# yeyupiaoling/MASR

Hardware: AMD Instinct MI355X
Metric: audio-seconds/sec (RTF^-1), conformer_streaming_fbank b32x10s, PCM->fbank->encoder->ctc_greedy->text (higher is better)
Workload: dtype f32; 1 GPU; configs[1]: conformer.yml streaming fbank, batch=32 synthetic 16 kHz 10 s utterances per GPU, ctc_greedy, random-init weights V=4233; global_batch=32, parallelism=dp1, world_size_observed=1, backend=none

## Files before the change

### include/masr_hip.h

```cpp
#ifndef MASR_HIP_H
#define MASR_HIP_H
#include <stdint.h>
#ifdef __cplusplus
extern "C" {
#endif

typedef struct masr_engine masr_engine;

typedef struct masr_config {
    int32_t model_kind;
    int32_t d_model;
    int32_t heads;
    int32_t d_ff;
    int32_t num_blocks;
    int32_t cnn_kernel;
    int32_t n_mels;
    int32_t vocab_size;
    int32_t causal;
    int32_t max_pos;
    int32_t device_id;
    int32_t reserved[5];
} masr_config;

const char* masr_last_error(void);
// ... 132 lines not shown

int masr_resample_f32(const float* x, int64_t n_orig, double ratio, const double* win, const double* dwin, int64_t nwin,
                      int32_t num_table, float* y, int64_t n_out);
int masr_encode_chunk(masr_engine* e, const int32_t* stream_ids, int32_t n, const float* feats_dev, int32_t Tc,
                      float* probs_dev, int32_t* argmax_dev, float* maxprob_dev, void* stream);
int masr_stream_export_cache(masr_engine* e, int32_t stream_id, float* att_dev, float* cnn_dev, void* stream);

int masr_op_layernorm(masr_engine* e, const float* x_dev, const float* w_dev, const float* b_dev, float* y_dev,
                      int32_t M, float eps, void* stream);
int masr_op_gemm(masr_engine* e, const float* a_dev, const float* w_dev, const float* bias_dev, const float* res_dev,
                 float* c_dev, int32_t M, int32_t N, int32_t K, int32_t act, float alpha, void* stream);

#define MASR_SIDE_STREAMS 5
int masr_side_stream(masr_engine* e, int32_t kind, void** stream_out);

#define MASR_LANES 2
int masr_select_lane(masr_engine* e, int32_t lane);

int masr_debug_set(masr_engine* e, int32_t key, int32_t value);

int masr_profile_select(masr_engine* e, int32_t kind);
int masr_profile_read(masr_engine* e, double* total_ms, int64_t* launches, double* flops, int32_t reset);

#ifdef __cplusplus
}
#endif
#endif
```

### masr_amd/_lib.py

```python
import ctypes as C
import os

from .build import LIB_PATH

_lib = None


class MasrConfig(C.Structure):
    _fields_ = [('model_kind', C.c_int32), ('d_model', C.c_int32), ('heads', C.c_int32), ('d_ff', C.c_int32),
                ('num_blocks', C.c_int32), ('cnn_kernel', C.c_int32), ('n_mels', C.c_int32),
                ('vocab_size', C.c_int32), ('causal', C.c_int32), ('max_pos', C.c_int32), ('device_id', C.c_int32),
                ('reserved', C.c_int32 * 5)]


class MasrError(RuntimeError):
    pass


_P = C.c_void_p
_I = C.c_int32
_F = C.c_float

SIGNATURES = {
    'masr_last_error': [],
# ... 52 lines not shown
    'masr_pool_close': [_P, _I],
    'masr_pool_reset': [_P, _I],
    'masr_pool_step': [_P, _I, _P, _P, _P, _P, _P, _P, _P, C.POINTER(_I), C.POINTER(_P), C.POINTER(_P), C.POINTER(_P),
                       C.POINTER(_I), C.POINTER(_P), _P],
    'masr_pool_profile': [_P, C.POINTER(C.c_double), C.POINTER(C.c_int64), _I],
    'masr_encoder_frames': [_P, _I, C.POINTER(_I)],
    'masr_engine_info': [_P, C.POINTER(_I), C.POINTER(_I), C.POINTER(_I)],
    'masr_stream_open': [_P, _I, C.POINTER(_I)],
    'masr_stream_reset': [_P, _I],
    'masr_stream_close': [_P, _I],
    'masr_stream_offset': [_P, _I, C.POINTER(_I)],
    'masr_stream_cache_len': [_P, _I, C.POINTER(_I)],
    'masr_stream_room': [_P, _I, C.POINTER(_I)],
    'masr_resample_f32': [_P, C.c_int64, C.c_double, _P, _P, C.c_int64, _I, _P, C.c_int64],
    'masr_stream_set_history': [_P, _I, _I],
    'masr_encode_chunk': [_P, C.POINTER(_I), _I, _P, _I, _P, _P, _P, _P],
    'masr_stream_export_cache': [_P, _I, _P, _P, _P],
    'masr_op_layernorm': [_P, _P, _P, _P, _P, _I, _F, _P],
    'masr_op_gemm': [_P, _P, _P, _P, _P, _P, _I, _I, _I, _I, _F, _P],
    'masr_side_stream': [_P, _I, C.POINTER(_P)],
    'masr_select_lane': [_P, _I],
    'masr_stage_rows': [_P, C.c_int64, _P, _P, _I, _I, _I],
    'masr_debug_set': [_P, _I, _I],
    'masr_profile_select': [_P, _I],
    'masr_profile_read': [_P, C.POINTER(C.c_double), C.POINTER(C.c_int64), C.POINTER(C.c_double), _I],
}
_RESTYPE = {'masr_last_error': C.c_char_p, 'masr_destroy': None, 'masr_beam_destroy': None, 'masr_lm_destroy': None,
            'masr_lm_last_error': C.c_char_p, 'masr_vad_last_error': C.c_char_p, 'masr_vad_destroy': None, 'masr_pool_destroy': None}


GAIN_FN = C.CFUNCTYPE(C.c_int, C.POINTER(C.c_float), C.c_int32, C.c_float, C.POINTER(C.c_float), C.c_void_p)


def lib():
    global _lib
    if _lib is not None:
        return _lib
    import torch
    if not os.path.exists(LIB_PATH):
        raise MasrError(f'{LIB_PATH} not found: build it with `python -m masr_amd.build` '
                        f'(hipcc --offload-arch=gfx950). There is no CPU fallback.')
    h = C.CDLL(LIB_PATH)
    for name, args in SIGNATURES.items():
        fn = getattr(h, name)
        fn.argtypes = args
        fn.restype = _RESTYPE.get(name, C.c_int)
# ... 8 lines not shown
```

### masr_amd/csrc/common.h

```cpp
#pragma once
#include <hip/hip_runtime.h>
#include <stdint.h>

#include "lm_scorer.h"

#ifndef MASR_EXPERIMENTS
#define MASR_EXPERIMENTS 0
#endif

typedef float f32x4 __attribute__((ext_vector_type(4)));
typedef float f32x16 __attribute__((ext_vector_type(16)));

namespace masr {

struct LdsAttr {
    size_t granted[32] = {};
};
void ensure_dynamic_lds(const void* fn, size_t bytes, LdsAttr& st);
void note_launch_error(const char* what, hipError_t e);

#ifdef __HIPCC__
struct SeqRow {
    int b, t;
};
// ... 168 lines not shown
    const float* pre_lnb;
    long plane_stride;
    int seq_t, pad_t;
};
struct FfnHead {
    const float* glu;
    const float* dw_w;
    const float* dw_b;
    const float* lnw;
    const float* lnb;
    const float* gconst;
    const float* W;
    const float* bias;
    const int* lens;
    int seq_t, ktaps, mstride;
    float* xout;
};
int launch_ffn_fused(float* x, const float* lnw, const float* lnb, const float* w1, const float* b1, const float* w2,
                     const float* b2, int M, int dff, float eps, float scale, int affine_prologue, float* partial,
                     int nsplit, hipStream_t s, const FfnPostLn* post = nullptr, const FfnTail* tail = nullptr,
                     const FfnHead* head = nullptr, bool packed = false);
void launch_pack_ffn_pc(const float* w1, const float* w2, float* p1, float* p2, int dff, hipStream_t s);
void launch_pack_rows_pc(const float* w, float* p, int N, hipStream_t s, int n_src = -1);
struct SqzStageArgs {
    float* x;
    float* out;
    const float* att;
    const float* head_w;
    const float* head_b;
    const float *ln_a_w, *ln_a_b, *ln_b_w, *ln_b_b;
    const float *ffn_s, *ffn_b, *w1, *b1, *w2, *b2;
    const float *tail_w, *tail_b, *tail_s, *tail_sb;
    float* tail_out;
    float* glu_out;
    const float* glu;
    const float *dw_w, *dw_b, *bn_scale, *bn_shift, *gconst;
    const float* gpad;
    const int* lens;
    int M, dff, seq_t, mstride, ktaps, tail_n, glu_pad_l, glu_pad_tot;
    float eps;
    int skip_pad;
};
bool launch_sqz_stage(const SqzStageArgs& a, int stage, hipStream_t s);
#if MASR_EXPERIMENTS
int launch_ffn_dual(float* x, const float* lnw, const float* lnb, const float* p1, const float* b1, const float* p2,
                    const float* b2, int M, int dff, float eps, float scale, int affine_prologue, hipStream_t s,
// ... 134 lines not shown
```

### masr_amd/csrc/engine.hip

```cpp
#include <math.h>
#include <stdio.h>
#include <stdlib.h>
#include <string.h>

#include <map>
#include <mutex>
#include <string>
#include <vector>

#include "../../include/masr_hip.h"
#include "common.h"

using namespace masr;
namespace masr {
int lm_device_view(masr_lm* lm, LmView* out);
bool lm_word_based(const masr_lm* lm);
}
extern "C" const char* masr_lm_last_error(void);

static thread_local std::string g_err;
static int fail(const std::string& m) {
    g_err = m;
    return 1;
}
// ... 206 lines not shown
    int lane = 0;
    hipEvent_t pack_ev = nullptr;
    void* pack_stream = nullptr;
    bool pack_pending = false;
    bool finalized = false;
    std::map<std::string, HostTensor> host;
    std::vector<void*> owned;
    float *cmvn_mean = nullptr, *cmvn_istd = nullptr, *conv1_w = nullptr, *conv1_b = nullptr, *conv2_w = nullptr,
          *conv2_b = nullptr, *embed_w = nullptr, *embed_b = nullptr, *after_w = nullptr, *after_b = nullptr,
          *ctc_w = nullptr, *ctc_b = nullptr, *pe = nullptr;
    std::vector<LayerW> layers;
    std::vector<SqLayerW> sq_layers;
    std::vector<Ds2LayerW> ds2_layers;
    std::vector<GBeam> gbeams;
    DevBuf beam_pool, beam_state;
    std::map<void*, std::pair<DevBuf, DevBuf>> beam_ws;
    std::map<void*, DevBuf> ms_ws;
    int skip_padding = 7;
    void* beam_first_stream = nullptr;
    bool beam_first_set = false;
    std::map<const float*, std::pair<DevBuf, DevBuf>> ffn_packed;
    std::map<const float*, std::pair<DevBuf, DevBuf>> ffn_dual_packed;
    std::map<const float*, std::pair<DevBuf, DevBuf>> x3_packed;
    long long* beam_prof = nullptr;
    float *preln_w = nullptr, *preln_b = nullptr, *tr_dw_w = nullptr, *tr_dw_b = nullptr, *tr_pw_w = nullptr,
          *tr_pw_b = nullptr, *rec_w = nullptr, *rec_b = nullptr;
    int reduce_idx = -1, recover_idx = -1;
    int stride_idx = -1, n_group_layers = 0, group_size = 3;
    bool conv_bn = false;
    float *window = nullptr, *melwt = nullptr, *tw512 = nullptr, *twr4 = nullptr;
    FbankTables fbank_tables() const { return FbankTables{window, melwt, tw512, twr4, mel_lo}; }
    int* mel_lo = nullptr;
    float *dct = nullptr, *lifter = nullptr;
    int dct_ceps = 0;
    double *lin_win = nullptr, *lin_tw = nullptr;
    double lin_scale = 0.0;
    std::vector<Stream> streams;
    int prof_kind = 0;
    int prof_stride = 1, prof_seen = 0;
    std::vector<std::pair<hipEvent_t, hipEvent_t>> prof_events;
    size_t prof_used = 0;
    double prof_flops = 0.0;
};

namespace {

// ... 33 lines not shown
        on = e->prof_kind != 0 && (e->prof_kind == kind || (e->prof_kind == PROF_GEMM && (kind == PROF_FFN1 || kind == PROF_CONV2 || kind == PROF_FFN_TAIL || kind == PROF_FFN_HEAD)));
        if (on && e->prof_stride > 1) on = (e->prof_seen++ % e->prof_stride) == 0;
        if (!on) return;
        if (e->prof_used == e->prof_events.size()) {
            hipEvent_t a, b;
            hipEventCreate(&a);
            hipEventCreate(&b);
            e->prof_events.push_back({a, b});
        }
        hipEventRecord(e->prof_events[e->prof_used].first, s);
        e->prof_flops += flops;
    }
    ~ProfScope() {
        if (!on) return;
        hipEventRecord(e->prof_events[e->prof_used].second, s);
        e->prof_used++;
    }
};

struct CallGuard {
    masr_engine* e;
    hipStream_t s;
    size_t n0;
    static size_t packed_count(const masr_engine* e) { return e->ffn_packed.size() + e->ffn_dual_packed.size() + e->x3_packed.size(); }
    CallGuard(masr_engine* e_, hipStream_t s_) : e(e_), s(s_), n0(packed_count(e_)) {
        if (!e->pack_pending) return;
        if (hipEventQuery(e->pack_ev) == hipSuccess) {
            e->pack_pending = false;
        } else {
            (void)hipGetLastError();
            if ((void*)s != e->pack_stream) (void)hipStreamWaitEvent(s, e->pack_ev, 0);
        }
    }
    ~CallGuard() {
        if (packed_count(e) == n0) return;
        if (!e->pack_ev && hipEventCreateWithFlags(&e->pack_ev, hipEventDisableTiming) != hipSuccess) return;
        if (hipEventRecord(e->pack_ev, s) == hipSuccess) {
            e->pack_stream = (void*)s;
            e->pack_pending = true;
        }
    }
};

static int g_ffn_dual = 0;
static int g_ffn_packed = 2;
static int g_bf16x3 = 0;

void gemm(masr_engine* e, hipStream_t s, const float* A, int lda, const float* W, const float* bias, float* C, int ldc,
          int M, int N, int K, int act, float alpha, const float* R, int ldr, int kind = PROF_GEMM,
          const int* lens = nullptr, int mask_tp = 0) {
    GemmArgs a{};
    a.A = A; a.W = W; a.bias = bias; a.C = C; a.R = R; a.lens = lens;
    a.M = M; a.N = N; a.K = K; a.lda = lda; a.ldc = ldc; a.ldr = ldr;
    a.act = act; a.alpha = alpha; a.mask_tp = mask_tp;
    ProfScope ps(e, s, kind, 2.0 * M * (double)N * K);
    if (g_bf16x3 && launch_gemm_bf16x3(a, A_PLAIN, s)) return;
    launch_gemm(a, A_PLAIN, EPI_STD, s);
}

static int g_rowgemm_packed = 1;
const float* packed_rows_of(masr_engine* e, const float* W, int N, hipStream_t s) {
    auto it = e->ffn_packed.find(W);
    if (it == e->ffn_packed.end()) {
        const int Np = (N + 255) / 256 * 256;
        std::pair<DevBuf, DevBuf> pk;
        if (pk.first.ensure((size_t)Np * 256 * sizeof(float))) return nullptr;
        launch_pack_rows_pc(W, pk.first.as<float>(), Np, s, N);
        it = e->ffn_packed.emplace(W, pk).first;
// ... 233 lines not shown
        s.cnn2.release();
    }
    for (auto& g : e->gbeams) {
        g.pool.release();
        g.state.release();
    }
    for (auto& kv : e->beam_ws) {
        kv.second.first.release();
        kv.second.second.release();
    }
    for (auto& kv : e->ms_ws) kv.second.release();
    for (auto& kv : e->x3_packed) {
        kv.second.first.release();
        kv.second.second.release();
    }
    for (auto& kv : e->ffn_packed) {
        kv.second.first.release();
        kv.second.second.release();
    }
    for (auto& kv : e->ffn_dual_packed) {
        kv.second.first.release();
        kv.second.second.release();
    }
    for (auto& ev : e->prof_events) {
        (void)hipEventDestroy(ev.first);
        (void)hipEventDestroy(ev.second);
    }
    delete e;
}

static void drop_packed_weights(masr_engine* e) {
    if (e->ffn_packed.empty() && e->ffn_dual_packed.empty() && e->x3_packed.empty()) return;
    (void)hipSetDevice(e->cfg.device_id);
    (void)hipDeviceSynchronize();
    for (auto* m : {&e->ffn_packed, &e->ffn_dual_packed, &e->x3_packed}) {
        for (auto& kv : *m) {
            kv.second.first.release();
            kv.second.second.release();
        }
        m->clear();
    }
}

int masr_load_tensor(masr_engine* e, const char* name, const float* host, const int64_t* shape, int32_t ndim) {
    if (!e || !name || !host) return fail("null argument");
    std::string n(name);
    if (n.rfind("encoder.", 0) != 0 && n.rfind("ctc.", 0) != 0 && n.rfind("decoder.ctc_lo.", 0) != 0 && n != "__pos_table__")
        return 0;
    drop_packed_weights(e);
    HostTensor t;
    int64_t cnt = 1;
    for (int i = 0; i < ndim; ++i) {
        t.shape.push_back(shape[i]);
        cnt *= shape[i];
    }
    t.v.assign(host, host + cnt);
    e->host[n] = std::move(t);
    e->finalized = false;
// ... 235 lines not shown
            CHK(pk.first.ensure((size_t)dff * d * sizeof(float)));
            CHK(pk.second.ensure((size_t)dff * d * sizeof(float)));
            launch_pack_ffn_pc(w1, w2, pk.first.as<float>(), pk.second.as<float>(), dff, s);
            it = e->ffn_packed.emplace(w1, pk).first;
        }
        auto ic = e->ffn_dual_packed.find(w1 + 1);
        if (ic == e->ffn_dual_packed.end()) {
            std::pair<DevBuf, DevBuf> pk;
            CHK(pk.first.ensure((size_t)dff * d * sizeof(float)));
            launch_pack_ffn_coop_w1(w1, pk.first.as<float>(), dff, s);
            ic = e->ffn_dual_packed.emplace(w1 + 1, pk).first;
        }
        ProfScope psc(e, s, PROF_FFN1, 4.0 * M * (double)dff * d);
        launch_ffn_coop(e->x.as<float>(), lnw, lnb, ic->second.first.as<float>(), b1, it->second.second.as<float>(), M, dff, 1e-5f,
                        affine, e->ffpart.as<float>(), s);
        launch_ffn_reduce(e->x.as<float>(), e->ffpart.as<float>(), b2, M, nsplit, scale, s, post_y ? &post : nullptr);
        if (tail_done) *tail_done = false;
        return 0;
    }
    ProfScope ps(e, s, want_tail ? PROF_FFN_TAIL : want_head ? PROF_FFN_HEAD : PROF_FFN1,
                 4.0 * M * (double)dff * d + (want_tail ? 2.0 * M * (double)tail->N * d : 0.0) + (want_head ? 2.0 * M * (double)d * d : 0.0));
    const float *kw1 = w1, *kw2 = w2;
    const bool packed = g_ffn_packed && (nsplit == 1 || g_ffn_packed >= 2) && d == 256;
    if (packed) {
        auto it = e->ffn_packed.find(w1);
        if (it == e->ffn_packed.end()) {
            std::pair<DevBuf, DevBuf> pk;
            CHK(pk.first.ensure((size_t)dff * d * sizeof(float)));
            CHK(pk.second.ensure((size_t)dff * d * sizeof(float)));
            launch_pack_ffn_pc(w1, w2, pk.first.as<float>(), pk.second.as<float>(), dff, s);
            it = e->ffn_packed.emplace(w1, pk).first;
        }
        kw1 = it->second.first.as<float>();
        kw2 = it->second.second.as<float>();
    }
    FfnTail ptail{};
    FfnHead phead{};
    auto packed_rows = [&](const float* W, int N, const float** out) -> int {
        auto it = e->ffn_packed.find(W);
        if (it == e->ffn_packed.end()) {
            std::pair<DevBuf, DevBuf> pk;
            CHK(pk.first.ensure((size_t)N * d * sizeof(float)));
            launch_pack_rows_pc(W, pk.first.as<float>(), N, s);
            it = e->ffn_packed.emplace(W, pk).first;
        }
        *out = it->second.first.as<float>();
        return 0;
// ... 5 lines not shown
            CHK(pk.first.ensure((size_t)dff * d * sizeof(float)));
            CHK(pk.second.ensure((size_t)dff * d * sizeof(float)));
            launch_pack_ffn_dual(w1, w2, pk.first.as<float>(), pk.second.as<float>(), dff, s);
            it = e->ffn_dual_packed.emplace(w1, pk).first;
        }
        if (want_tail) {
            ptail = *tail;
            auto tw = e->ffn_dual_packed.find(tail->W);
            if (tw == e->ffn_dual_packed.end()) {
                std::pair<DevBuf, DevBuf> pk;
                CHK(pk.first.ensure((size_t)768 * d * sizeof(float)));
                launch_pack_rows_dual(tail->W, pk.first.as<float>(), s);
                tw = e->ffn_dual_packed.emplace(tail->W, pk).first;
            }
            ptail.W = tw->second.first.as<float>();
        }
        if (want_head) {
            phead = *head;
            CHK(packed_rows(head->W, d, &phead.W));
        }
        const int done = launch_ffn_dual(e->x.as<float>(), lnw, lnb, it->second.first.as<float>(), b1, it->second.second.as<float>(),
                                         b2, M, dff, 1e-5f, scale, affine, s, want_tail ? &ptail : nullptr, want_head ? &phead : nullptr);
        if (done < 0) return fail("ffn(): the two-chain FFN kernel rejected the launch");
        if (want_head && done != 4) return fail("ffn(): head stage was not launched");
        if (tail_done) *tail_done = done == 2;
        if (post_y) launch_layernorm(e->x.as<float>(), post_w, post_b, post_y, M, 1e-5f, 0, 0, nullptr, s);
        return 0;
    }
    if (packed && want_tail && tail->N % 256 == 0) {
        ptail = *tail;
        CHK(packed_rows(tail->W, tail->N, &ptail.W));
        tail = &ptail;
    }
    if (packed && want_head) {
        phead = *head;
        CHK(packed_rows(head->W, d, &phead.W));
        if (split_head) {
            CHK(e->xh.ensure((size_t)M * d * sizeof(float)));
            phead.xout = e->xh.as<float>();
        }
        head = &phead;
    }
    const int done = launch_ffn_fused(e->x.as<float>(), lnw, lnb, kw1, b1, kw2, b2, M, dff, 1e-5f, scale, affine,
                                      nsplit > 1 ? e->ffpart.as<float>() : nullptr, nsplit, s, post_y ? &post : nullptr,
                                      want_tail ? tail : nullptr, want_head ? head : nullptr, packed);
    if (done < 0) return fail("ffn(): launch rejected");
// ... 1765 lines not shown
    else if (key == 7) set_attention_fewq(value);
    else if (key == 14) set_attention_fold(value);
    else if (key == 15) g_embed_split = value;
    else if (key == 19) g_hot_weights = value;
    else if (key == 20) g_bf16x3 = value;
    else if (key == 21) set_gemm_bf16x3_waves(value);
    else if (key == 22) set_ffn_x3_rotation(value);
    else if (key == 23) g_ffn_packed = value;
    else if (key == 24) g_ffn_dual = value;
    else if (key == 25) g_rowgemm_packed = value;
    else if (key == 26) set_attention_grouped_fold(value);
    else if (key == 27) g_ctc_fused_blocks = value;
    else if (key == 28) set_attention_fewq_wgs(value);
    else if (key == 29) g_few_rows_path = value;
    else if (key == 30) g_split_head = value;
    else if (key == 31) g_efficient_fused = value;
    else if (key == 32) g_beam_lm_cache = value;
    else if (key == 33) set_conv2_mid_fill(value);
    else if (key == 34) g_attn_chain = value;
    else if (key == 35) g_ffn_coop = value;
    else if (key == 36) g_sqz_fused_blocks = value;
    else if (key == 37) g_beam_narrow = value;
    else if (key == 38) e->skip_padding = value;
    else if (key == 17) set_gemm_waves(value);
    else if (key == 18) set_conv1_nt(value);
    else if (key == 16) { e->prof_stride = value > 1 ? value : 1; e->prof_seen = 0; }
    else if (key == 8) g_no_ffn_tail = value;
    else if (key == 9) g_no_ffn_head = value;
    else if (key == 12) set_rowgemm_small_blocks(value);
    else if (key == 13) g_ffn_split_blocks = value;
    else if (key == 2) {
        if (value) {
            if (!e->beam_prof) {
                void* p = nullptr;
                HIPCHK(hipMalloc(&p, 16 * sizeof(long long)));
                e->owned.push_back(p);
                e->beam_prof = (long long*)p;
            }
        } else if (e->beam_prof) {
            long long h[16];
            HIPCHK(hipMemcpy(h, e->beam_prof, sizeof(h), hipMemcpyDeviceToHost));
            fprintf(stderr, "beam phases (cycles, last workgroup): setup+hash %lld  extensions %lld  prefixes+count %lld  select %lld  compact %lld\n",
                    h[0], h[1], h[2], h[3], h[4]);
            fprintf(stderr, "  narrow step (%lld frames): tables+candidates %lld  hash+contexts %lld  children+scorer table %lld  extensions %lld  "
                    "prefixes+select %lld  scan %lld  survivors %lld  new prefixes %lld\n", h[5], h[6], h[7], h[8], h[9], h[10], h[11], h[12], h[13]);
            if (h[15] > 0) fprintf(stderr, "  wide step (%lld frames): %.1f distinct scorer contexts per frame\n", h[15], (double)h[14] / (double)h[15]);
// ... 35 lines not shown
```

### masr_amd/csrc/ffn_pc.hip

```cpp
#include "common.h"

namespace masr {

static constexpr int PC_BM = 32;
static constexpr int PC_D = 256;
static constexpr int PC_CH = 128;
static constexpr int PC_XLD = PC_D + 4;
static constexpr int PC_HLD = PC_CH + 4;
static constexpr int PC_WLD = 32 + 4;
static constexpr int PC_WSLAB = 32 * PC_WLD;
static constexpr int PC_NSET = 4;
#ifdef PC_NOFENCE_PACKED
#define PC_FENCE(var) do { if ((var) != 2) __builtin_amdgcn_sched_barrier(0); } while (0)
#else
#define PC_FENCE(var) __builtin_amdgcn_sched_barrier(0)
#endif

#ifndef PC_BUFLOAD
#define PC_BUFLOAD 1
#endif
__device__ __forceinline__ f32x4 pc_bufld(__amdgpu_buffer_rsrc_t rs, unsigned lane16, unsigned float_index) {
    return __builtin_bit_cast(f32x4, __builtin_amdgcn_raw_buffer_load_b128(rs, lane16, float_index * 4u, 0));
}

// ... 495 lines not shown
                }
            }
            if (col < tail.N && tail.plane_stride > 0) {
                float* plane = tail.out + (size_t)t * tail.plane_stride + wave * 32 + frow;
                const int pb0 = row0 / tail.seq_t, pt0 = row0 - pb0 * tail.seq_t;
#pragma unroll
                for (int r = 0; r < 16; ++r) {
                    const int lr = (r & 3) + 8 * (r >> 2) + 4 * fh;
                    const SeqRow q = seq_row(pb0, pt0, tail.seq_t, lr);
                    if (row0 + lr < M) plane[((size_t)q.b * (tail.seq_t + tail.pad_t) + q.t) * 256] = acc[r] + bv;
                }
            } else if (col < tail.N) {
#pragma unroll
                for (int r = 0; r < 16; ++r) {
                    const int row = row0 + (r & 3) + 8 * (r >> 2) + 4 * fh;
                    if (row < M) tail.out[(size_t)row * tail.ldo + col] = acc[r] + bv;
                }
            }
        }
    }
}


__global__ __launch_bounds__(256) void pack_ffn_pc_kernel(const float* __restrict__ w1, const float* __restrict__ w2,
                                                          float* __restrict__ p1, float* __restrict__ p2, int dff) {
    const size_t n = (size_t)dff * PC_D;
    const size_t t = (size_t)blockIdx.x * 256 + threadIdx.x;
    if (t >= 2 * n) return;
    const bool second = t >= n;
    const size_t e = second ? t - n : t;
    const int q = (int)(e & 3), lane = (int)((e >> 2) & 63), g = (int)((e >> 8) & 3), j = (int)((e >> 10) & 7),
              idx = (int)((e >> 13) & 3), chunk = (int)(e >> 15);
    const int frow = lane & 31, fh = lane >> 5;
    if (!second) p1[e] = w1[(size_t)(chunk * PC_CH + 32 * idx + frow) * PC_D + 32 * j + 8 * g + 4 * fh + q];
    else p2[e] = w2[(size_t)(64 * idx + 32 * (j & 1) + frow) * dff + chunk * PC_CH + 32 * (j >> 1) + 8 * g + 4 * fh + q];
}
__global__ __launch_bounds__(256) void pack_rows_pc_kernel(const float* __restrict__ w, float* __restrict__ p, int N, int n_src) {
    const size_t e = (size_t)blockIdx.x * 256 + threadIdx.x;
    if (e >= (size_t)N * PC_D) return;
    const int q = (int)(e & 3), lane = (int)((e >> 2) & 63), g = (int)((e >> 8) & 3), j = (int)((e >> 10) & 7),
              wave = (int)((e >> 13) & 7), t = (int)(e >> 16);
    const int row = t * 256 + 32 * wave + (lane & 31);
    p[e] = row < n_src ? w[(size_t)row * PC_D + 32 * j + 8 * g + 4 * (lane >> 5) + q] : 0.f;
}
void launch_pack_rows_pc(const float* w, float* p, int N, hipStream_t s, int n_src) {
    const size_t n = (size_t)N * PC_D;
// ... 51 lines not shown
    } else if (tail && tail->out && tail->N % 256 == 0 && !AFFINE && VAR != 1) {
        hipLaunchKernelGGL((ffn_pc_kernel<0, 0, TV, 1, 0>), dim3((M + PC_BM - 1) / PC_BM), dim3(512), lds, s, x, lnw, lnb, w1, b1, w2,
                           b2, M, dff, eps, scale, (float*)nullptr, 0, *tail, FfnHead{});
        return 2;
    } else {
        hipLaunchKernelGGL((ffn_pc_kernel<AFFINE, 0, VAR, 0, 0>), dim3((M + PC_BM - 1) / PC_BM), dim3(512), lds, s, x, lnw, lnb, w1,
                           b1, w2, b2, M, dff, eps, scale, (float*)nullptr, 0, FfnTail{}, FfnHead{});
    }
    return 0;
}

int launch_ffn_pc(float* x, const float* lnw, const float* lnb, const float* w1, const float* b1, const float* w2,
                  const float* b2, int M, int dff, float eps, float scale, int affine_prologue, float* partial, int nsplit,
                  hipStream_t s, int variant, const FfnPostLn* post, const FfnTail* tail, const FfnHead* head) {
    if (M <= 0) return 0;
    if (affine_prologue && variant == 2) return launch_pc_t<1, 2>(x, lnw, lnb, w1, b1, w2, b2, M, dff, eps, scale, partial, nsplit, s, post, nullptr, nullptr);
    if (affine_prologue) return launch_pc_t<1, 0>(x, lnw, lnb, w1, b1, w2, b2, M, dff, eps, scale, partial, nsplit, s, post, nullptr, nullptr);
    if (variant == 1) return launch_pc_t<0, 1>(x, lnw, lnb, w1, b1, w2, b2, M, dff, eps, scale, partial, nsplit, s, post, nullptr, nullptr);
    if (variant == 2) return launch_pc_t<0, 2>(x, lnw, lnb, w1, b1, w2, b2, M, dff, eps, scale, partial, nsplit, s, post, tail, head);
    return launch_pc_t<0, 0>(x, lnw, lnb, w1, b1, w2, b2, M, dff, eps, scale, partial, nsplit, s, post, tail, head);
}

}
```

Measured before the change: 49800 audio-seconds/sec.

## Add 16-row-tile FFN kernel using 16x16x4 MFMA with new weight packing

Adds a new fused FFN kernel that processes 16 rows per block using 16x16x4 f32 MFMA instead of the 32-row 32x32x2 path. It comes with a matching weight-packing layout and supports the fused head (depthwise conv) and tail stages. It is enabled by default for unsplit, non-affine d=256 FFNs. The smaller row tile is meant to give more blocks for the modest M in this workload and better occupancy. The trade-off is less weight reuse per block and more weight traffic. An MFMA accumulation-order probe kernel is also exported to check numerical equivalence of the two orders.

```diff
diff --git a/include/masr_hip.h b/include/masr_hip.h
--- a/include/masr_hip.h
+++ b/include/masr_hip.h
@@ -178,6 +178,9 @@
 int masr_profile_select(masr_engine* e, int32_t kind);
 int masr_profile_read(masr_engine* e, double* total_ms, int64_t* launches, double* flops, int32_t reset);
 
+int masr_mfma_order_probe(const float* a_dev, const float* b_dev, float* c32_dev, float* c16_dev, int32_t k, const int32_t* perm,
+                          void* stream);
+
 #ifdef __cplusplus
 }
 #endif
diff --git a/masr_amd/_lib.py b/masr_amd/_lib.py
--- a/masr_amd/_lib.py
+++ b/masr_amd/_lib.py
@@ -98,6 +98,7 @@
     'masr_select_lane': [_P, _I],
     'masr_stage_rows': [_P, C.c_int64, _P, _P, _I, _I, _I],
     'masr_debug_set': [_P, _I, _I],
+    'masr_mfma_order_probe': [_P, _P, _P, _P, _I, _P, _P],
     'masr_profile_select': [_P, _I],
     'masr_profile_read': [_P, C.POINTER(C.c_double), C.POINTER(C.c_int64), C.POINTER(C.c_double), _I],
 }
diff --git a/masr_amd/csrc/common.h b/masr_amd/csrc/common.h
--- a/masr_amd/csrc/common.h
+++ b/masr_amd/csrc/common.h
@@ -214,6 +214,10 @@
                      const FfnHead* head = nullptr, bool packed = false);
 void launch_pack_ffn_pc(const float* w1, const float* w2, float* p1, float* p2, int dff, hipStream_t s);
 void launch_pack_rows_pc(const float* w, float* p, int N, hipStream_t s, int n_src = -1);
+int launch_ffn16(float* x, const float* lnw, const float* lnb, const float* w1, const float* b1, const float* w2, const float* b2, int M,
+                 int dff, float eps, float scale, hipStream_t s, const FfnTail* tail, const FfnHead* head);
+void launch_pack_ffn16(const float* w1, const float* w2, float* p1, float* p2, int dff, hipStream_t s);
+void launch_pack_rows16(const float* w, float* p, int N, hipStream_t s, int n_src = -1);
 struct SqzStageArgs {
     float* x;
     float* out;
diff --git a/masr_amd/csrc/engine.hip b/masr_amd/csrc/engine.hip
--- a/masr_amd/csrc/engine.hip
+++ b/masr_amd/csrc/engine.hip
@@ -252,6 +252,7 @@
     std::map<const float*, std::pair<DevBuf, DevBuf>> ffn_packed;
     std::map<const float*, std::pair<DevBuf, DevBuf>> ffn_dual_packed;
     std::map<const float*, std::pair<DevBuf, DevBuf>> x3_packed;
+    std::map<const float*, std::pair<DevBuf, DevBuf>> ffn16_packed;
     long long* beam_prof = nullptr;
     float *preln_w = nullptr, *preln_b = nullptr, *tr_dw_w = nullptr, *tr_dw_b = nullptr, *tr_pw_w = nullptr,
           *tr_pw_b = nullptr, *rec_w = nullptr, *rec_b = nullptr;
@@ -331,7 +332,9 @@
     masr_engine* e;
     hipStream_t s;
     size_t n0;
-    static size_t packed_count(const masr_engine* e) { return e->ffn_packed.size() + e->ffn_dual_packed.size() + e->x3_packed.size(); }
+    static size_t packed_count(const masr_engine* e) {
+        return e->ffn_packed.size() + e->ffn_dual_packed.size() + e->x3_packed.size() + e->ffn16_packed.size();
+    }
     CallGuard(masr_engine* e_, hipStream_t s_) : e(e_), s(s_), n0(packed_count(e_)) {
         if (!e->pack_pending) return;
         if (hipEventQuery(e->pack_ev) == hipSuccess) {
@@ -353,6 +356,7 @@
 
 static int g_ffn_dual = 0;
 static int g_ffn_packed = 2;
+static int g_ffn16 = 1;
 static int g_bf16x3 = 0;
 
 void gemm(masr_engine* e, hipStream_t s, const float* A, int lda, const float* W, const float* bias, float* C, int ldc,
@@ -632,6 +636,10 @@
         kv.second.first.release();
         kv.second.second.release();
     }
+    for (auto& kv : e->ffn16_packed) {
+        kv.second.first.release();
+        kv.second.second.release();
+    }
     for (auto& ev : e->prof_events) {
         (void)hipEventDestroy(ev.first);
         (void)hipEventDestroy(ev.second);
@@ -640,10 +648,10 @@
 }
 
 static void drop_packed_weights(masr_engine* e) {
-    if (e->ffn_packed.empty() && e->ffn_dual_packed.empty() && e->x3_packed.empty()) return;
+    if (e->ffn_packed.empty() && e->ffn_dual_packed.empty() && e->x3_packed.empty() && e->ffn16_packed.empty()) return;
     (void)hipSetDevice(e->cfg.device_id);
     (void)hipDeviceSynchronize();
-    for (auto* m : {&e->ffn_packed, &e->ffn_dual_packed, &e->x3_packed}) {
+    for (auto* m : {&e->ffn_packed, &e->ffn_dual_packed, &e->x3_packed, &e->ffn16_packed}) {
         for (auto& kv : *m) {
             kv.second.first.release();
             kv.second.second.release();
@@ -925,7 +933,9 @@
                  4.0 * M * (double)dff * d + (want_tail ? 2.0 * M * (double)tail->N * d : 0.0) + (want_head ? 2.0 * M * (double)d * d : 0.0));
     const float *kw1 = w1, *kw2 = w2;
     const bool packed = g_ffn_packed && (nsplit == 1 || g_ffn_packed >= 2) && d == 256;
-    if (packed) {
+    const bool use16 = packed && nsplit == 1 && g_ffn16 && !affine && dff % 128 == 0 && !(want_tail && tail->N % 256) &&
+                       !(want_head && head->ktaps != 15 && head->ktaps != 7);
+    if (packed && !use16) {
         auto it = e->ffn_packed.find(w1);
         if (it == e->ffn_packed.end()) {
             std::pair<DevBuf, DevBuf> pk;
@@ -977,6 +987,42 @@
         const int done = launch_ffn_dual(e->x.as<float>(), lnw, lnb, it->second.first.as<float>(), b1, it->second.second.as<float>(),
                                          b2, M, dff, 1e-5f, scale, affine, s, want_tail ? &ptail : nullptr, want_head ? &phead : nullptr);
         if (done < 0) return fail("ffn(): the two-chain FFN kernel rejected the launch");
+        if (want_head && done != 4) return fail("ffn(): head stage was not launched");
+        if (tail_done) *tail_done = done == 2;
+        if (post_y) launch_layernorm(e->x.as<float>(), post_w, post_b, post_y, M, 1e-5f, 0, 0, nullptr, s);
+        return 0;
+    }
+    if (use16) {
+        auto p16 = [&](const float* W, int N, const float** out) -> int {
+            auto it = e->ffn16_packed.find(W);
+            if (it == e->ffn16_packed.end()) {
+                std::pair<DevBuf, DevBuf> pk;
+                CHK(pk.first.ensure((size_t)N * d * sizeof(float)));
+                launch_pack_rows16(W, pk.first.as<float>(), N, s);
+                it = e->ffn16_packed.emplace(W, pk).first;
+            }
+            *out = it->second.first.as<float>();
+            return 0;
+        };
+        auto it = e->ffn16_packed.find(w1);
+        if (it == e->ffn16_packed.end()) {
+            std::pair<DevBuf, DevBuf> pk;
+            CHK(pk.first.ensure((size_t)dff * d * sizeof(float)));
+            CHK(pk.second.ensure((size_t)dff * d * sizeof(float)));
+            launch_pack_ffn16(w1, w2, pk.first.as<float>(), pk.second.as<float>(), dff, s);
+            it = e->ffn16_packed.emplace(w1, pk).first;
+        }
+        if (want_tail) {
+            ptail = *tail;
+            CHK(p16(tail->W, tail->N, &ptail.W));
+        }
+        if (want_head) {
+            phead = *head;
+            CHK(p16(head->W, d, &phead.W));
+        }
+        const int done = launch_ffn16(e->x.as<float>(), lnw, lnb, it->second.first.as<float>(), b1, it->second.second.as<float>(), b2, M,
+                                      dff, 1e-5f, scale, s, want_tail ? &ptail : nullptr, want_head ? &phead : nullptr);
+        if (done < 0) return fail("ffn(): the 16-row FFN kernel rejected the launch");
         if (want_head && done != 4) return fail("ffn(): head stage was not launched");
         if (tail_done) *tail_done = done == 2;
         if (post_y) launch_layernorm(e->x.as<float>(), post_w, post_b, post_y, M, 1e-5f, 0, 0, nullptr, s);
@@ -2788,6 +2834,7 @@
     else if (key == 36) g_sqz_fused_blocks = value;
     else if (key == 37) g_beam_narrow = value;
     else if (key == 38) e->skip_padding = value;
+    else if (key == 39) g_ffn16 = value;
     else if (key == 17) set_gemm_waves(value);
     else if (key == 18) set_conv1_nt(value);
     else if (key == 16) { e->prof_stride = value > 1 ? value : 1; e->prof_seen = 0; }
diff --git a/masr_amd/csrc/ffn_pc.hip b/masr_amd/csrc/ffn_pc.hip
--- a/masr_amd/csrc/ffn_pc.hip
+++ b/masr_amd/csrc/ffn_pc.hip
@@ -541,6 +541,446 @@
 }
 
 
+static constexpr int P16_BM = 16;
+static constexpr int P16_RING = 8;
+__host__ __device__ constexpr int p16_k0(int kk) { return (kk & 1) * 4 + (kk >> 1); }
+
+template <int TAIL, int HEADK>
+__global__ __launch_bounds__(512) __attribute__((amdgpu_waves_per_eu(4))) void ffn16_kernel(
+    float* x, const float* __restrict__ lnw, const float* __restrict__ lnb, const float* __restrict__ w1, const float* __restrict__ b1,
+    const float* __restrict__ w2, const float* __restrict__ b2, int M, int dff, float eps, float scale, FfnTail tail, FfnHead head) {
+    extern __shared__ __align__(16) float sm[];
+    float* xn = sm;
+    float* hs = xn + P16_BM * PC_XLD;
+
+    const int tid = threadIdx.x, lane = tid & 63;
+    const int wave = __builtin_amdgcn_readfirstlane(tid >> 6);
+    const int role = wave >> 2, idx = wave & 3;
+    const int row0 = blockIdx.x * P16_BM;
+    const int fr = lane & 15, kk = lane >> 4, ko = p16_k0(kk);
+    const unsigned lane16 = lane * 16;
+    f32x4 pre[P16_RING];
+    const float* xa = xn + fr * PC_XLD + ko;
+
+    f32x4 gw_head = {0.f, 0.f, 0.f, 0.f}, gb_head = gw_head;
+    if (HEADK > 0) {
+        {
+            constexpr int KT = HEADK > 0 ? HEADK : 1, pad = KT - 1;
+            const int c = tid & 255, half = tid >> 8;
+            float w[KT], win[KT], nw[8];
+#pragma unroll
+            for (int j = 0; j < KT; ++j) w[j] = head.dw_w[j * 256 + c];
+            const float bv = head.dw_b[c];
+            const float gc = head.gconst ? head.gconst[c] : 0.f;
+            const bool has_gc = head.gconst != nullptr;
+            const int hb0 = row0 / head.seq_t, ht0 = row0 - hb0 * head.seq_t, lr_last = M - 1 - row0;
+#pragma unroll
+            for (int rr = 0; rr < 8; ++rr) {
+                const SeqRow q = seq_row(hb0, ht0, head.seq_t, min(half * 8 + rr, lr_last));
+                nw[rr] = head.glu[((size_t)q.b * (pad + head.seq_t) + q.t + pad) * 256 + c];
+            }
+#pragma unroll
+            for (int j = 0; j < KT; ++j) win[j] = 0.f;
+#pragma unroll
+            for (int rr = 0; rr < 8; ++rr) {
+                const int lr = half * 8 + rr;
+                const SeqRow q = seq_row(hb0, ht0, head.seq_t, min(lr, lr_last));
+                const int b = q.b, t = q.t;
+                if (rr == 0 || t == 0 || row0 + lr >= M) {
+                    const float* gin = head.glu + ((size_t)b * (pad + head.seq_t) + t) * 256 + c;
+#pragma unroll
+                    for (int j = 0; j < pad; ++j) win[j + 1] = (has_gc && t + j < pad) ? gc : gin[(size_t)j * 256];
+                }
+#pragma unroll
+                for (int j = 0; j < pad; ++j) win[j] = win[j + 1];
+                win[pad] = nw[rr];
+                float acc = bv;
+#pragma unroll
+                for (int j = 0; j < KT; ++j) acc = fmaf(w[j], win[j], acc);
+                xn[lr * PC_XLD + c] = acc;
+            }
+        }
+        {
+            const f32x4 ww = *reinterpret_cast<const f32x4*>(head.lnw + lane * 4);
+            const f32x4 bb = *reinterpret_cast<const f32x4*>(head.lnb + lane * 4);
+            __syncthreads();
+#pragma unroll
+            for (int rr = 0; rr < 2; ++rr) {
+                const int lr = wave * 2 + rr;
+                const f32x4 v = *reinterpret_cast<const f32x4*>(&xn[lr * PC_XLD + lane * 4]);
+                const float mean = pc_wsum(v[0] + v[1] + v[2] + v[3]) * (1.0f / 256.0f);
+                const float d0 = v[0] - mean, d1 = v[1] - mean, d2 = v[2] - mean, d3 = v[3] - mean;
+                const float var = pc_wsum(d0 * d0 + d1 * d1 + d2 * d2 + d3 * d3) * (1.0f / 256.0f);
+                const float rstd = 1.0f / sqrtf(var + eps);
+                f32x4 o;
+                o[0] = d0 * rstd * ww[0] + bb[0];
+                o[1] = d1 * rstd * ww[1] + bb[1];
+                o[2] = d2 * rstd * ww[2] + bb[2];
+                o[3] = d3 * rstd * ww[3] + bb[3];
+#pragma unroll
+                for (int i = 0; i < 4; ++i) o[i] = o[i] / (1.0f + expf(-o[i]));
+                *reinterpret_cast<f32x4*>(&xn[lr * PC_XLD + lane * 4]) = o;
+            }
+        }
+        const __amdgpu_buffer_rsrc_t hrs = __builtin_amdgcn_make_buffer_rsrc(const_cast<float*>(head.W), 0, PC_D * PC_D * 4, 0x00020000);
+        auto hld = [&](int f) -> f32x4 { return pc_bufld(hrs, lane16, (unsigned)(wave * 32 + f) * 256u); };
+#pragma unroll
+        for (int k = 0; k < P16_RING; ++k) pre[k] = hld(k);
+        __syncthreads();
+        {
+            float bv[2], res[8];
+            unsigned padded = 0;
+            const int mb0 = row0 / head.seq_t, mt0 = row0 - mb0 * head.seq_t;
+#pragma unroll
+            for (int nt = 0; nt < 2; ++nt) {
+                const int col = wave * 32 + 16 * nt + fr;
+                bv[nt] = head.bias[col];
+#pragma unroll
+                for (int r = 0; r < 4; ++r) {
+                    const int lrc = min(4 * kk + r, M - 1 - row0);
+                    res[4 * nt + r] = x[(size_t)(row0 + lrc) * PC_D + col];
+                    if (head.lens) {
+                        const SeqRow q = seq_row(mb0, mt0, head.seq_t, lrc);
+                        if (head.mstride * q.t >= head.lens[q.b]) padded |= 1u << (4 * nt + r);
+                    }
+                }
+            }
+            gw_head = *reinterpret_cast<const f32x4*>(lnw + lane * 4);
+            gb_head = *reinterpret_cast<const f32x4*>(lnb + lane * 4);
+            f32x4 acc[2] = {{0.f, 0.f, 0.f, 0.f}, {0.f, 0.f, 0.f, 0.f}};
+            float a0 = xa[0], a1 = xa[2];
+#pragma unroll
+            for (int g = 0; g < 32; ++g) {
+                float n0 = 0.f, n1 = 0.f;
+                if (g + 1 < 32) { n0 = xa[8 * (g + 1)]; n1 = xa[8 * (g + 1) + 2]; }
+#pragma unroll
+                for (int q = 0; q < 4; ++q) {
+                    acc[q & 1] = __builtin_amdgcn_mfma_f32_16x16x4f32(q < 2 ? a0 : a1, pre[g % P16_RING][q], acc[q & 1], 0, 0, 0);
+                    if (q == 3 && g + P16_RING < 32) pre[g % P16_RING] = hld(g + P16_RING);
+                    __builtin_amdgcn_sched_barrier(0);
+                }
+                a0 = n0;
+                a1 = n1;
+            }
+            __syncthreads();
+#pragma unroll
+            for (int nt = 0; nt < 2; ++nt) {
+                const int col = wave * 32 + 16 * nt + fr;
+#pragma unroll
+                for (int r = 0; r < 4; ++r) {
+                    const int lr = 4 * kk + r;
+                    float v = acc[nt][r] + bv[nt];
+                    if (padded & (1u << (4 * nt + r))) v = 0.f;
+                    v = res[4 * nt + r] + v;
+                    if (row0 + lr < M) x[(size_t)(row0 + lr) * PC_D + col] = v;
+                    xn[lr * PC_XLD + col] = v;
+                }
+            }
+        }
+        __syncthreads();
+    }
+
+    {
+        const f32x4 gw = HEADK > 0 ? gw_head : *reinterpret_cast<const f32x4*>(lnw + lane * 4);
+        const f32x4 gb = HEADK > 0 ? gb_head : *reinterpret_cast<const f32x4*>(lnb + lane * 4);
+        f32x4 v4[2];
+#pragma unroll
+        for (int rr = 0; rr < 2; ++rr) {
+            const int row = min(row0 + wave * 2 + rr, M - 1);
+            v4[rr] = HEADK > 0 ? *reinterpret_cast<const f32x4*>(&xn[(wave * 2 + rr) * PC_XLD + lane * 4])
+                               : *reinterpret_cast<const f32x4*>(x + (size_t)row * PC_D + lane * 4);
+        }
+        if (TAIL && tail.pre_lnw) {
+            const f32x4 pw = *reinterpret_cast<const f32x4*>(tail.pre_lnw + lane * 4);
+            const f32x4 pb = *reinterpret_cast<const f32x4*>(tail.pre_lnb + lane * 4);
+#pragma unroll
+            for (int rr = 0; rr < 2; ++rr) {
+                const f32x4 v = v4[rr];
+                const float mean = pc_wsum(v[0] + v[1] + v[2] + v[3]) * (1.0f / 256.0f);
+                const float d0 = v[0] - mean, d1 = v[1] - mean, d2 = v[2] - mean, d3 = v[3] - mean;
+                const float var = pc_wsum(d0 * d0 + d1 * d1 + d2 * d2 + d3 * d3) * (1.0f / 256.0f);
+                const float rstd = 1.0f / sqrtf(var + eps);
+                f32x4 o;
+                o[0] = d0 * rstd * pw[0] + pb[0];
+                o[1] = d1 * rstd * pw[1] + pb[1];
+                o[2] = d2 * rstd * pw[2] + pb[2];
+                o[3] = d3 * rstd * pw[3] + pb[3];
+                v4[rr] = o;
+                const int row = row0 + wave * 2 + rr;
+                if (row < M) *reinterpret_cast<f32x4*>(x + (size_t)row * PC_D + lane * 4) = o;
+            }
+        }
+#pragma unroll
+        for (int rr = 0; rr < 2; ++rr) {
+            const int lr = wave * 2 + rr;
+            const f32x4 v = v4[rr];
+            const float mean = pc_wsum(v[0] + v[1] + v[2] + v[3]) * (1.0f / 256.0f);
+            const float d0 = v[0] - mean, d1 = v[1] - mean, d2 = v[2] - mean, d3 = v[3] - mean;
+            const float var = pc_wsum(d0 * d0 + d1 * d1 + d2 * d2 + d3 * d3) * (1.0f / 256.0f);
+            const float rstd = 1.0f / sqrtf(var + eps);
+            f32x4 o;
+            o[0] = d0 * rstd * gw[0] + gb[0];
+            o[1] = d1 * rstd * gw[1] + gb[1];
+            o[2] = d2 * rstd * gw[2] + gb[2];
+            o[3] = d3 * rstd * gw[3] + gb[3];
+            if (row0 + lr >= M) o = f32x4{0.f, 0.f, 0.f, 0.f};
+            *reinterpret_cast<f32x4*>(&xn[lr * PC_XLD + lane * 4]) = o;
+        }
+    }
+
+    const int nchunk = dff / PC_CH, nlast = nchunk - 1;
+    const __amdgpu_buffer_rsrc_t wrs = __builtin_amdgcn_make_buffer_rsrc(const_cast<float*>(role == 0 ? w1 : w2), 0, dff * PC_D * 4, 0x00020000);
+    auto pld = [&](int chunk, int f) -> f32x4 { return pc_bufld(wrs, lane16, (unsigned)((chunk * 4 + idx) * 32 + f) * 256u); };
+#pragma unroll
+    for (int k = 0; k < P16_RING; ++k) pre[k] = pld(0, k);
+    __syncthreads();
+
+    if (role == 0) {
+        f32x4 accp[2] = {{0.f, 0.f, 0.f, 0.f}, {0.f, 0.f, 0.f, 0.f}};
+        float bvp[2] = {0.f, 0.f};
+        f32x4 resx[4];
+        for (int phase = 0; phase <= nchunk + 1; ++phase) {
+            float* hprev = hs + ((phase + 1) & 1) * P16_BM * PC_HLD + idx * 32 + fr;
+            auto finish = [&](int e) {
+                const int nt = e >> 2, r = e & 3;
+                const float v = accp[nt][r] + bvp[nt];
+                hprev[(4 * kk + r) * PC_HLD + 16 * nt] = v * __builtin_amdgcn_rcpf(1.0f + __expf(-v));
+            };
+            if (phase < nchunk) {
+                const int chunk = phase;
+                const float bv0 = b1[chunk * PC_CH + idx * 32 + fr], bv1 = b1[chunk * PC_CH + idx * 32 + 16 + fr];
+                f32x4 acc[2] = {{0.f, 0.f, 0.f, 0.f}, {0.f, 0.f, 0.f, 0.f}};
+                float a0 = xa[0], a1 = xa[2];
+#pragma unroll
+                for (int g = 0; g < 32; ++g) {
+                    float n0 = 0.f, n1 = 0.f;
+                    if (g + 1 < 32) { n0 = xa[8 * (g + 1)]; n1 = xa[8 * (g + 1) + 2]; }
+#pragma unroll
+                    for (int q = 0; q < 4; ++q) {
+                        acc[q & 1] = __builtin_amdgcn_mfma_f32_16x16x4f32(q < 2 ? a0 : a1, pre[g % P16_RING][q], acc[q & 1], 0, 0, 0);
+                        if (q == 3) pre[g % P16_RING] = pld(min(chunk + (g + P16_RING) / 32, nlast), (g + P16_RING) & 31);
+                        if (phase > 0 && q == 1 && (g & 3) == 1) finish(g >> 2);
+                        __builtin_amdgcn_sched_barrier(0);
+                    }
+                    a0 = n0;
+                    a1 = n1;
+                }
+                accp[0] = acc[0];
+                accp[1] = acc[1];
+                bvp[0] = bv0;
+                bvp[1] = bv1;
+            } else if (phase == nchunk) {
+#pragma unroll
+                for (int e = 0; e < 8; ++e) finish(e);
+#pragma unroll
+                for (int i = 0; i < 4; ++i) {
+                    const int row = min(row0 + idx * 4 + i, M - 1);
+                    resx[i] = *reinterpret_cast<const f32x4*>(x + (size_t)row * PC_D + lane * 4);
+                }
+            } else {
+#pragma unroll
+                for (int i = 0; i < 4; ++i) *reinterpret_cast<f32x4*>(&xn[(idx * 4 + i) * PC_XLD + lane * 4]) = resx[i];
+            }
+            __syncthreads();
+        }
+    } else {
+        f32x4 acc2[4];
+#pragma unroll
+        for (int n = 0; n < 4; ++n) acc2[n] = f32x4{0.f, 0.f, 0.f, 0.f};
+        float bv2n[4];
+#pragma unroll
+        for (int n = 0; n < 4; ++n) bv2n[n] = b2[idx * 64 + 16 * n + fr];
+        for (int phase = 0; phase <= nchunk + 1; ++phase) {
+            if (phase >= 2) {
+                const int chunk = phase - 2;
+                const float* ha = hs + (phase & 1) * P16_BM * PC_HLD + fr * PC_HLD + ko;
+                float a = ha[0];
+#pragma unroll
+                for (int f = 0; f < 32; ++f) {
+                    const float an = f + 1 < 32 ? ha[8 * ((f + 1) >> 1) + 2 * ((f + 1) & 1)] : 0.f;
+#pragma unroll
+                    for (int q = 0; q < 4; ++q) {
+                        acc2[q] = __builtin_amdgcn_mfma_f32_16x16x4f32(a, pre[f % P16_RING][q], acc2[q], 0, 0, 0);
+                        if (q == 3) pre[f % P16_RING] = pld(min(chunk + (f + P16_RING) / 32, nlast), (f + P16_RING) & 31);
+                        __builtin_amdgcn_sched_barrier(0);
+                    }
+                    a = an;
+                }
+            }
+            __syncthreads();
+        }
+#pragma unroll
+        for (int n = 0; n < 4; ++n) {
+            const int col = idx * 64 + 16 * n + fr;
+            const float bv2 = bv2n[n];
+#pragma unroll
+            for (int r = 0; r < 4; ++r) {
+                const int lr = 4 * kk + r;
+                const float v = xn[lr * PC_XLD + col] + scale * (acc2[n][r] + bv2);
+                if (row0 + lr < M) x[(size_t)(row0 + lr) * PC_D + col] = v;
+                if (TAIL) xn[lr * PC_XLD + col] = v;
+            }
+        }
+    }
+    if (!TAIL) return;
+
+    {
+        const f32x4 gw = *reinterpret_cast<const f32x4*>(tail.lnw + lane * 4);
+        const f32x4 gb = *reinterpret_cast<const f32x4*>(tail.lnb + lane * 4);
+        __syncthreads();
+#pragma unroll
+        for (int rr = 0; rr < 2; ++rr) {
+            const int lr = wave * 2 + rr;
+            const f32x4 v = *reinterpret_cast<const f32x4*>(&xn[lr * PC_XLD + lane * 4]);
+            const float mean = pc_wsum(v[0] + v[1] + v[2] + v[3]) * (1.0f / 256.0f);
+            const float d0 = v[0] - mean, d1 = v[1] - mean, d2 = v[2] - mean, d3 = v[3] - mean;
+            const float var = pc_wsum(d0 * d0 + d1 * d1 + d2 * d2 + d3 * d3) * (1.0f / 256.0f);
+            const float rstd = 1.0f / sqrtf(var + eps);
+            f32x4 o;
+            o[0] = d0 * rstd * gw[0] + gb[0];
+            o[1] = d1 * rstd * gw[1] + gb[1];
+            o[2] = d2 * rstd * gw[2] + gb[2];
+            o[3] = d3 * rstd * gw[3] + gb[3];
+            if (row0 + lr >= M) o = f32x4{0.f, 0.f, 0.f, 0.f};
+            *reinterpret_cast<f32x4*>(&xn[lr * PC_XLD + lane * 4]) = o;
+        }
+    }
+    const int ntile = (tail.N + 255) / 256;
+    const __amdgpu_buffer_rsrc_t trs = __builtin_amdgcn_make_buffer_rsrc(const_cast<float*>(tail.W), 0, ntile * 256 * PC_D * 4, 0x00020000);
+    auto tld = [&](int t, int f) -> f32x4 { return pc_bufld(trs, lane16, (unsigned)((min(t, ntile - 1) * 8 + wave) * 32 + f) * 256u); };
+#pragma unroll
+    for (int k = 0; k < P16_RING; ++k) pre[k] = tld(0, k);
+    __syncthreads();
+    for (int t = 0; t < ntile; ++t) {
+        float bv[2];
+#pragma unroll
+        for (int nt = 0; nt < 2; ++nt) bv[nt] = tail.bias[min(t * 256 + wave * 32 + 16 * nt + fr, tail.N - 1)];
+        f32x4 acc[2] = {{0.f, 0.f, 0.f, 0.f}, {0.f, 0.f, 0.f, 0.f}};
+        float a0 = xa[0], a1 = xa[2];
+#pragma unroll
+        for (int g = 0; g < 32; ++g) {
+            float n0 = 0.f, n1 = 0.f;
+            if (g + 1 < 32) { n0 = xa[8 * (g + 1)]; n1 = xa[8 * (g + 1) + 2]; }
+#pragma unroll
+            for (int q = 0; q < 4; ++q) {
+                acc[q & 1] = __builtin_amdgcn_mfma_f32_16x16x4f32(q < 2 ? a0 : a1, pre[g % P16_RING][q], acc[q & 1], 0, 0, 0);
+                if (q == 3) pre[g % P16_RING] = tld(t + (g + P16_RING) / 32, (g + P16_RING) & 31);
+                __builtin_amdgcn_sched_barrier(0);
+            }
+            a0 = n0;
+            a1 = n1;
+        }
+#pragma unroll
+        for (int nt = 0; nt < 2; ++nt) {
+            const int col = t * 256 + wave * 32 + 16 * nt + fr;
+            if (col >= tail.N) continue;
+            if (tail.plane_stride > 0) {
+                float* plane = tail.out + (size_t)t * tail.plane_stride + wave * 32 + 16 * nt + fr;
+                const int pb0 = row0 / tail.seq_t, pt0 = row0 - pb0 * tail.seq_t;
+#pragma unroll
+                for (int r = 0; r < 4; ++r) {
+                    const int lr = 4 * kk + r;
+                    const SeqRow q = seq_row(pb0, pt0, tail.seq_t, lr);
+                    if (row0 + lr < M) plane[((size_t)q.b * (tail.seq_t + tail.pad_t) + q.t) * 256] = acc[nt][r] + bv[nt];
+                }
+            } else {
+#pragma unroll
+                for (int r = 0; r < 4; ++r) {
+                    const int row = row0 + 4 * kk + r;
+                    if (row < M) tail.out[(size_t)row * tail.ldo + col] = acc[nt][r] + bv[nt];
+                }
+            }
+        }
+    }
+}
+
+__global__ __launch_bounds__(256) void pack_ffn16_kernel(const float* __restrict__ w1, const float* __restrict__ w2,
+                                                         float* __restrict__ p1, float* __restrict__ p2, int dff) {
+    const size_t n = (size_t)dff * PC_D;
+    const size_t t = (size_t)blockIdx.x * 256 + threadIdx.x;
+    if (t >= 2 * n) return;
+    const bool second = t >= n;
+    const size_t e = second ? t - n : t;
+    const int q = (int)(e & 3), lane = (int)((e >> 2) & 63), f = (int)((e >> 8) & 31), idx = (int)((e >> 13) & 3), chunk = (int)(e >> 15);
+    const int fr = lane & 15, ko = p16_k0(lane >> 4);
+    if (!second) p1[e] = w1[(size_t)(chunk * PC_CH + 32 * idx + 16 * (q & 1) + fr) * PC_D + 8 * f + ko + 2 * (q >> 1)];
+    else p2[e] = w2[(size_t)(64 * idx + 16 * q + fr) * dff + chunk * PC_CH + 8 * (f >> 1) + ko + 2 * (f & 1)];
+}
+__global__ __launch_bounds__(256) void pack_rows16_kernel(const float* __restrict__ w, float* __restrict__ p, int N, int n_src) {
+    const size_t e = (size_t)blockIdx.x * 256 + threadIdx.x;
+    if (e >= (size_t)N * PC_D) return;
+    const int q = (int)(e & 3), lane = (int)((e >> 2) & 63), f = (int)((e >> 8) & 31), wave = (int)((e >> 13) & 7), t = (int)(e >> 16);
+    const int row = t * 256 + 32 * wave + 16 * (q & 1) + (lane & 15);
+    p[e] = row < n_src ? w[(size_t)row * PC_D + 8 * f + p16_k0(lane >> 4) + 2 * (q >> 1)] : 0.f;
+}
+void launch_pack_ffn16(const float* w1, const float* w2, float* p1, float* p2, int dff, hipStream_t s) {
+    const size_t n = (size_t)2 * dff * PC_D;
+    hipLaunchKernelGGL(pack_ffn16_kernel, dim3((unsigned)((n + 255) / 256)), dim3(256), 0, s, w1, w2, p1, p2, dff);
+}
+void launch_pack_rows16(const float* w, float* p, int N, hipStream_t s, int n_src) {
+    const size_t n = (size_t)N * PC_D;
+    hipLaunchKernelGGL(pack_rows16_kernel, dim3((unsigned)((n + 255) / 256)), dim3(256), 0, s, w, p, N, n_src < 0 ? N : n_src);
+}
+
+int launch_ffn16(float* x, const float* lnw, const float* lnb, const float* w1, const float* b1, const float* w2, const float* b2, int M,
+                 int dff, float eps, float scale, hipStream_t s, const FfnTail* tail, const FfnHead* head) {
+    if (M <= 0) return 0;
+    if (dff % PC_CH || dff <= 0 || (tail && tail->out && head && head->glu)) return -1;
+    const size_t lds = (size_t)(P16_BM * PC_XLD + 2 * P16_BM * PC_HLD) * sizeof(float);
+    const dim3 grid((M + P16_BM - 1) / P16_BM);
+    if (head && head->glu) {
+        if (head->ktaps == 15)
+            hipLaunchKernelGGL((ffn16_kernel<0, 15>), grid, dim3(512), lds, s, x, lnw, lnb, w1, b1, w2, b2, M, dff, eps, scale, FfnTail{}, *head);
+        else if (head->ktaps == 7)
+            hipLaunchKernelGGL((ffn16_kernel<0, 7>), grid, dim3(512), lds, s, x, lnw, lnb, w1, b1, w2, b2, M, dff, eps, scale, FfnTail{}, *head);
+        else
+            return -1;
+        return 4;
+    }
+    if (tail && tail->out) {
+        if (tail->N % 256) return -1;
+        hipLaunchKernelGGL((ffn16_kernel<1, 0>), grid, dim3(512), lds, s, x, lnw, lnb, w1, b1, w2, b2, M, dff, eps, scale, *tail, FfnHead{});
+        return 2;
+    }
+    hipLaunchKernelGGL((ffn16_kernel<0, 0>), grid, dim3(512), lds, s, x, lnw, lnb, w1, b1, w2, b2, M, dff, eps, scale, FfnTail{}, FfnHead{});
+    return 0;
+}
+
+__global__ __launch_bounds__(64) void mfma_order_probe_kernel(const float* __restrict__ a, const float* __restrict__ b, float* c32,
+                                                              float* c16, int K, int4 p0, int4 p1) {
+    const int lane = threadIdx.x;
+    {
+        const int frow = lane & 31, fh = lane >> 5;
+        f32x16 acc;
+#pragma unroll
+        for (int r = 0; r < 16; ++r) acc[r] = 0.f;
+        for (int g = 0; g < K / 8; ++g)
+#pragma unroll
+            for (int q = 0; q < 4; ++q) {
+                const int k = 8 * g + 4 * fh + q;
+                const float av = frow < 16 ? a[frow * K + k] : 0.f, bv = frow < 16 ? b[frow * K + k] : 0.f;
+                acc = __builtin_amdgcn_mfma_f32_32x32x2f32(av, bv, acc, 0, 0, 0);
+            }
+#pragma unroll
+        for (int r = 0; r < 16; ++r) {
+            const int row = (r & 3) + 8 * (r >> 2) + 4 * fh;
+            if (row < 16 && frow < 16) c32[row * 16 + frow] = acc[r];
+        }
+    }
+    {
+        const int fr = lane & 15, kk = lane >> 4;
+        const int o0 = kk == 0 ? p0.x : kk == 1 ? p0.y : kk == 2 ? p0.z : p0.w;
+        const int o1 = kk == 0 ? p1.x : kk == 1 ? p1.y : kk == 2 ? p1.z : p1.w;
+        f32x4 acc = {0.f, 0.f, 0.f, 0.f};
+        for (int g = 0; g < K / 8; ++g) {
+            acc = __builtin_amdgcn_mfma_f32_16x16x4f32(a[fr * K + 8 * g + o0], b[fr * K + 8 * g + o0], acc, 0, 0, 0);
+            acc = __builtin_amdgcn_mfma_f32_16x16x4f32(a[fr * K + 8 * g + o1], b[fr * K + 8 * g + o1], acc, 0, 0, 0);
+        }
+#pragma unroll
+        for (int r = 0; r < 4; ++r) c16[(4 * kk + r) * 16 + fr] = acc[r];
+    }
+}
+
 __global__ __launch_bounds__(256) void pack_ffn_pc_kernel(const float* __restrict__ w1, const float* __restrict__ w2,
                                                           float* __restrict__ p1, float* __restrict__ p2, int dff) {
     const size_t n = (size_t)dff * PC_D;
@@ -638,3 +1078,13 @@
 }
 
 }
+
+extern "C" int masr_mfma_order_probe(const float* a_dev, const float* b_dev, float* c32_dev, float* c16_dev, int32_t k,
+                                     const int32_t* perm, void* stream) {
+    if (!a_dev || !b_dev || !c32_dev || !c16_dev || !perm || k <= 0 || k % 8) return 1;
+    for (int i = 0; i < 8; ++i)
+        if (perm[i] < 0 || perm[i] > 7) return 1;
+    hipLaunchKernelGGL(masr::mfma_order_probe_kernel, dim3(1), dim3(64), 0, (hipStream_t)stream, a_dev, b_dev, c32_dev, c16_dev, (int)k,
+                       make_int4(perm[0], perm[1], perm[2], perm[3]), make_int4(perm[4], perm[5], perm[6], perm[7]));
+    return hipGetLastError() == hipSuccess ? 0 : 1;
+}
```

After: 51190 audio-seconds/sec (median of 6 runs). +2.8%, better.
